# jaymarichua/Applestar

Hardware: AMD Instinct MI355X
Metric: learner samples/sec (AlphaStar policy) (higher is better)
Workload: dtype fp32

## Files before the change

applestar_amd/csrc/bindings.cpp:

```cpp
#include <cstring>
#include <cstdlib>
#include <map>
#include <string>
#include <torch/extension.h>
#include <c10/hip/HIPStream.h>
#include <c10/hip/HIPGuard.h>

#include "kernels.h"

namespace {

hipStream_t stream() { return c10::hip::getCurrentHIPStream().stream(); }

int dt(const at::Tensor& t) {
  if (t.scalar_type() == at::kFloat) return as::DT_F32;
  if (t.scalar_type() == at::kBFloat16) return as::DT_BF16;
  TORCH_CHECK(false, "applestar_amd: unsupported dtype ", t.scalar_type());
}

void check_cuda(const at::Tensor& t, const char* name) {
  TORCH_CHECK(t.is_cuda(), "applestar_amd: ", name, " must be a GPU tensor");
  TORCH_CHECK(t.is_contiguous(), "applestar_amd: ", name, " must be contiguous");
}

// ... 2298 lines not shown
    const at::Tensor& s = srcs[i];
    TORCH_CHECK(d.is_cuda() && s.is_cuda() && d.device() == s.device(), "multi_strided_copy: GPU tensors");
    TORCH_CHECK(d.is_contiguous(), "multi_strided_copy: contiguous destination");
    TORCH_CHECK((d.scalar_type() == at::kFloat || d.scalar_type() == at::kBFloat16) &&
                (s.scalar_type() == at::kFloat || s.scalar_type() == at::kBFloat16), "multi_strided_copy: fp32/bf16");
    const int64_t* sp = spec.data() + 9 * i;
    int64_t n = 1, lo = sp[8], hi = sp[8];
    for (int k = 0; k < 4; ++k) {
      TORCH_CHECK(sp[k] >= 1, "multi_strided_copy: sizes >= 1");
      n *= sp[k];
      const int64_t reach = (sp[k] - 1) * sp[4 + k];
      if (reach < 0) lo += reach; else hi += reach;
    }
    TORCH_CHECK(n == d.numel() && n < (int64_t{1} << 31), "multi_strided_copy: spec / destination size");
    int64_t extent = 1;
    for (int64_t k = 0; k < s.dim(); ++k) extent += (s.size(k) - 1) * s.stride(k);
    TORCH_CHECK(lo >= 0 && hi < extent, "multi_strided_copy: spec reaches outside the source");
    const int t = a.ntensors++;
    a.src[t] = s.data_ptr();
    a.dst[t] = d.data_ptr();
    a.n[t] = static_cast<int>(n);
    for (int k = 0; k < 4; ++k) {
      a.size[t][k] = static_cast<int>(sp[k]);
      a.stride[t][k] = sp[4 + k];
    }
    a.base[t] = sp[8];
    const bool tiled = sp[0] == 1 && sp[1] == 1 && sp[6] == 1 && sp[7] > 1 && n >= (1 << 16);
    a.dts[t] = static_cast<unsigned char>((s.scalar_type() == at::kFloat ? 1 : 0) | (d.scalar_type() == at::kFloat ? 2 : 0) |
                                          (tiled ? 4 : 0));
    const int64_t chunks = tiled ? ((sp[2] + 63) / 64) * ((sp[3] + 127) / 128) : (n + as::kCopyChunk - 1) / as::kCopyChunk;
    a.chunk_start[t + 1] = a.chunk_start[t] + static_cast<int>(chunks);
    if (a.ntensors == as::kSCopyMaxT) flush();
  }
  flush();
}

at::Tensor pointwise_conv(const at::Tensor& x, const at::Tensor& w, const c10::optional<at::Tensor>& bias, int64_t act) {
  check_cuda(x, "x");
  check_cuda(w, "w");
  TORCH_CHECK(x.scalar_type() == at::kBFloat16 && x.dim() == 2, "pointwise: x [P, cin] bf16");
  TORCH_CHECK(w.scalar_type() == at::kFloat && w.dim() == 2 && w.size(1) == x.size(1), "pointwise: w fp32 [cout, cin]");
  const int64_t P = x.size(0), cin = x.size(1), cout = w.size(0);
  TORCH_CHECK(as::pointwise_supported(static_cast<int>(cin), static_cast<int>(cout)), "pointwise: channels");
  const float* bp = nullptr;
  if (bias.has_value()) {
    check_cuda(*bias, "bias");
    TORCH_CHECK(bias->scalar_type() == at::kFloat && bias->numel() == cout, "pointwise: bias fp32 [cout]");
    bp = bias->data_ptr<float>();
  }
  c10::hip::HIPGuard g(x.device().index());
  auto y = at::empty({P, cout}, x.options());
  as::pointwise_conv(x.data_ptr(), w.data_ptr<float>(), bp, y.data_ptr(), P, static_cast<int>(cin),
                     static_cast<int>(cout), static_cast<int>(act), stream());
  return y;
}

void register_codec(pybind11::module& m);

PYBIND11_MODULE(TORCH_EXTENSION_NAME, m) {
  m.doc() = "applestar_amd HIP kernels for gfx950 (MI355X)";
  register_codec(m);
  m.def("layer_norm_fwd", &layer_norm_fwd);
  m.def("layer_norm_bwd", &layer_norm_bwd, py::arg("dy"), py::arg("xin"), py::arg("y"), py::arg("w"), py::arg("mean"),
        py::arg("rstd"), py::arg("dx_dtype"), py::arg("act"), py::arg("mask_src") = py::none());
  m.def("reverse_scan", &reverse_scan);
  m.def("col_sum", &col_sum);
  m.def("multi_logp", &multi_logp);
  m.def("presplit_b", &presplit_b, py::arg("b"), py::arg("trans") = false, py::arg("out") = py::none());
  m.def("gemm_f32_psb_supported", &gemm_f32_psb_supported);
  m.def("multi_presplit", &multi_presplit);
  m.def("conv3x3_f32_psb_supported", &conv3x3_f32_psb_supported);
  m.def("conv3x3_f32_psb", &conv3x3_f32_psb, py::arg("x"), py::arg("wsplit"), py::arg("Cout"),
        py::arg("bias") = py::none(), py::arg("res") = py::none(), py::arg("res2") = py::none(),
        py::arg("mask") = py::none(), py::arg("act") = 0);
  m.def("conv3x3_f32_v2", &conv3x3_f32_v2, py::arg("x"), py::arg("wsplit"), py::arg("Cout"),
        py::arg("bias") = py::none(), py::arg("res") = py::none(), py::arg("res2") = py::none(),
        py::arg("mask") = py::none(), py::arg("act") = 0, py::arg("variant") = 0);
  m.def("conv3x3_f32_halo_supported", &conv3x3_f32_halo_supported);
  m.def("conv3x3_f32_halo", &conv3x3_f32_halo, py::arg("x"), py::arg("wsplit"), py::arg("Cout"),
        py::arg("bias") = py::none(), py::arg("res") = py::none(), py::arg("res2") = py::none(),
        py::arg("mask") = py::none(), py::arg("act") = 0);
  m.def("conv_halo_f32_mode", &as::conv_halo_f32_mode);
  m.def("set_conv_halo_f32_mode", &as::set_conv_halo_f32_mode);
  m.def("gemm_f32_psb", &gemm_f32_psb, py::arg("a"), py::arg("bsplit"), py::arg("N"), py::arg("K"),
        py::arg("bias") = py::none(), py::arg("res") = py::none(), py::arg("act") = 0, py::arg("variant") = 0);
  m.def("entity_pack", &entity_pack);
  m.def("embed_relu_fwd", &embed_relu_fwd);
  m.def("embed_relu_bwd", &embed_relu_bwd, py::arg("dout"), py::arg("out"), py::arg("idx"), py::arg("V"),
        py::arg("ordered") = false);
  m.def("gated_residual_fwd", &gated_residual_fwd, py::arg("y"), py::arg("g"), py::arg("sp"), py::arg("x"),
        py::arg("post") = py::none());
  m.def("gated_residual_bwd", &gated_residual_bwd, py::arg("dout"), py::arg("y"), py::arg("g"), py::arg("sp"),
        py::arg("out"), py::arg("xin") = py::none());
  m.def("lnlstm_fwd", &lnlstm_fwd, py::arg("xp"), py::arg("h0"), py::arg("c0"), py::arg("wT"),
        py::arg("lnh_w"), py::arg("lnh_b"), py::arg("lnc_w"), py::arg("lnc_b"),
        py::arg("eps"), py::arg("want_bf16") = false);
  m.def("lnlstm_bwd", &lnlstm_bwd);
  m.def("entity_embed_fwd", &entity_embed_fwd);
  m.def("entity_onehot", &entity_onehot);
  m.def("upsample2x_fwd", &upsample2x_fwd);
  m.def("upsample2x_bwd", &upsample2x_bwd, py::arg("dy"), py::arg("mask") = py::none());
  m.def("entity_embed_wgrad", &entity_embed_wgrad);
  m.def("mm_k32", &mm_k32);
  m.def("spatial_embed_fwd", &spatial_embed_fwd, py::arg("planes"), py::arg("effects"), py::arg("w_dense"),
        py::arg("bias"), py::arg("rows"), py::arg("ex"), py::arg("ey"), py::arg("entity_num"), py::arg("out_dtype"),
        py::arg("ordered") = false);
  m.def("spatial_gather_rows", &spatial_gather_rows, py::arg("dpre"), py::arg("ex"), py::arg("ey"),
        py::arg("entity_num"), py::arg("N"), py::arg("gate") = py::none());
  m.def("spatial_dense_input", &spatial_dense_input);
  m.def("spatial_dense_wgrad", &spatial_dense_wgrad, py::arg("planes"), py::arg("effects"), py::arg("dpre"),
        py::arg("gate") = py::none());
  m.def("varlen_attn_fwd", &varlen_attn_fwd);
  m.def("varlen_attn_bwd", &varlen_attn_bwd);
  m.def("varlen_attn_fwd_f32", &varlen_attn_fwd_f32);
  m.def("conv3x3_f32_epi2", &conv3x3_f32_epi2);
  m.def("conv3x3_f32_epi2_supported", &conv3x3_f32_epi2_supported);
  m.def("conv3x3_f32", &conv3x3_f32);
  m.def("fused_clip_adam", &fused_clip_adam);
  m.def("head_sample", &head_sample);
  m.def("target_unit_sample", &target_unit_sample);
  m.def("fused_adam_chunk", &as::fused_adam_chunk);
  m.def("wgrad_f32", &wgrad_f32, py::arg("dy"), py::arg("x"), py::arg("cin"), py::arg("want_bias"),
        py::arg("out") = py::none());
  m.def("gemm_f32", &gemm_f32);
  m.def("gemm_bf16_small", &gemm_bf16_small);
  m.def("gemm_bf16", &gemm_bf16);
  m.def("small_gemm", &small_gemm);
  m.def("small_wgrad", &small_wgrad);
  m.def("small_gemm_splitk", &small_gemm_splitk);
  m.def("f32_mfma_mode", &as::f32_mfma_mode);
  m.def("set_f32_pipe_variant", &as::set_f32_pipe_variant);
  m.def("set_f32_conv_variant", &as::set_f32_conv_variant);
  m.def("set_f32_mfma_mode", &as::set_f32_mfma_mode);
  m.def("conv3x3_f32_supported", &as::conv3x3_f32_supported);
  m.def("varlen_attn_bwd_f32", &varlen_attn_bwd_f32);
  m.def("attn_f32_variant", [](int64_t v) { return static_cast<int64_t>(as::attn_f32_variant(static_cast<int>(v))); });
  m.def("su_sample", &su_sample);
  m.def("segment_copy", &segment_copy);
  m.def("conv_wt", &conv_wt);
  m.def("upconv1_fwd", &upconv1_fwd);
  m.def("upconv1_bwd", &upconv1_bwd, py::arg("x_nhwc"), py::arg("w"), py::arg("dy"), py::arg("relu_mask") = false);
  m.def("maxpool2_fwd", &maxpool2_fwd);
  m.def("maxpool2_bwd", &maxpool2_bwd, py::arg("dy"), py::arg("pos"), py::arg("H"), py::arg("W"),
        py::arg("mask") = py::none());
  m.def("maxpool2_bwd_relu", &maxpool2_bwd_relu);
  m.def("spatial_embed_pool_fwd", &spatial_embed_pool_fwd, py::arg("planes"), py::arg("effects"), py::arg("w_dense"),
        py::arg("bias"), py::arg("rows"), py::arg("ex"), py::arg("ey"), py::arg("entity_num"),
        py::arg("ordered") = false);
  m.def("spatial_pool_supported", [](int64_t h, int64_t w) { return as::spatial_pool_supported(static_cast<int>(h), static_cast<int>(w)); });
  m.def("segment_sum", &segment_sum);
  m.def("spatial_dense_wgrad_pooled", &spatial_dense_wgrad_pooled);
  m.def("spatial_gather_rows_pooled", &spatial_gather_rows_pooled);
  m.def("entity_mean_pool", &entity_mean_pool);
  m.def("table_grad", &table_grad, py::arg("src"), py::arg("idx"), py::arg("V"), py::arg("ordered") = false);
  m.def("gather_steps_fwd", &gather_steps_fwd);
  m.def("gather_steps_bwd", &gather_steps_bwd);
  m.def("scatter_conn_fwd", &scatter_conn_fwd);
  m.def("scatter_conn_bwd", &scatter_conn_bwd);
  m.def("conv3x3_fwd", &conv3x3_fwd);
  m.def("wgrad", &wgrad, py::arg("dy"), py::arg("x"), py::arg("cin"), py::arg("want_bias"),
        py::arg("bf16_out") = false);
  m.def("pointwise_conv", &pointwise_conv);
  m.def("pointwise_supported", [](int64_t ci, int64_t co) { return as::pointwise_supported(static_cast<int>(ci), static_cast<int>(co)); });
  m.def("lstm_split_error", &lstm_split_error);
  m.def("lstm_split_flag", &lstm_split_flag);
  m.def("multi_copy", &multi_copy);
// ... 29 lines not shown
```

applestar_amd/csrc/conv_tap.h:

```cpp
#pragma once
#include "common.h"

namespace as {

__device__ __forceinline__ int conv_tap_mask(long m, long M, int HW, int H, int W) {
  int ok = 0;
  if (m < M) {
    const int rem = static_cast<int>(m % HW);
    const int yy = rem / W, xx = rem - yy * W;
#pragma unroll
    for (int t = 0; t < 9; ++t) {
      const int y2 = yy + t / 3 - 1, x2 = xx + t % 3 - 1;
      ok |= (y2 >= 0 && y2 < H && x2 >= 0 && x2 < W) << t;
    }
  }
  return ok;
}

struct ConvTap {
  int tap, c0, shift;
  __device__ __forceinline__ bool in(int mask) const { return (mask >> tap) & 1; }
  __device__ __forceinline__ int offset(bool ok, int pix, int Cin, int c, int es) const {
    return ok ? ((pix + shift) * Cin + c0 + c) * es : kOOB;
  }
};

__device__ __forceinline__ ConvTap conv_tap(int k0, int Cin, int W) {
  const int tap = k0 / Cin;
  return ConvTap{tap, k0 - tap * Cin, (tap / 3 - 1) * W + (tap % 3 - 1)};
}

}
```

applestar_amd/csrc/kernels.h:

```cpp
#pragma once
#include <hip/hip_runtime.h>
#include <stdint.h>

namespace as {

enum DType : int { DT_F32 = 0, DT_BF16 = 1 };
enum SrcType : int { SRC_U8 = 0, SRC_I8 = 1, SRC_I16 = 2, SRC_I32 = 3, SRC_I64 = 4, SRC_F16 = 5, SRC_F32 = 6 };
enum FieldKind : int { FIELD_ONE_HOT = 0, FIELD_BINARY = 1, FIELD_SCALAR = 2 };

constexpr int kMaxFields = 40;
struct EntityFields {
  const void* ptr[kMaxFields];
  int dtype[kMaxFields];
  int kind[kMaxFields];
  int offset[kMaxFields];
  int width[kMaxFields];
  int n;
};

void layer_norm_fwd(const void* x, int x_dt, const void* res, int res_dt, const float* w, const float* b,
                    void* y, int y_dt, float* xsum, float* mean, float* rstd, long rows, int cols, float eps,
                    int act, hipStream_t s);
void layer_norm_bwd(const void* dy, int dy_dt, const void* xin, int xin_dt, const void* y, int y_dt,
                    const float* w, const float* mean, const float* rstd, void* dx, int dx_dt,
                    float* dw_part, float* db_part, long rows, int cols, int act, int nblk, hipStream_t s,
                    const float* msrc = nullptr, float* dxm = nullptr);
void column_reduce(const float* part, float* out, int nrows, int cols, hipStream_t s);
void entity_pack(const void* num, bool num64, int B, int N, long total, bool* valid, int64_t* flat, int64_t* seg,
                 int* cu, hipStream_t s);
void embed_relu_fwd(const void* table, int dt, const void* idx, int idt, void* out, long U, int V, int D,
                    hipStream_t s);
void embed_relu_bwd(const void* dout, const void* out, int dt, const void* idx, int idt, float* dtab, long U, int V,
                    int D, bool direct, hipStream_t s);
void column_reduce_bf16(const float* part, void* out, int nrows, int cols, hipStream_t s);
int layer_norm_bwd_blocks(long rows);

void reverse_scan(const float* a, const float* b, const float* init, float* y, int K, int T, int B,
                  hipStream_t s);

void gated_residual_fwd(const void* y, const void* g, const float* sp, const void* x, const void* post, void* out,
                        int dt, long n, hipStream_t s);
int vsp_in_channels();
int vsp_out_channels();
void vsp_fwd(const void* sc, const void* own, const void* enemy, const float* w, const float* b, void* out, long P,
             hipStream_t s, int dt = DT_BF16);
int vsp_bwd_blocks(long P);
void vsp_pool_fwd(const void* sc, const void* own, const void* enemy, const float* w, const float* b, void* pooled,
                  uint8_t* pos, int B, int H, int W, hipStream_t s, int dt = DT_BF16);
void vsp_pool_bwd(const void* dpooled, const uint8_t* pos, const void* pooled, const void* sc, const void* own,
                  const void* enemy, const float* w, void* dsc, float* part, int B, int H, int W, int nblk,
                  hipStream_t s, int dt = DT_BF16);
void vsp_bwd(const void* dout, const void* out, const void* sc, const void* own, const void* enemy, const float* w,
             void* dsc, float* part, long P, int nblk, hipStream_t s, int dt = DT_BF16);
bool loc_in_supported(int C, int P);
void loc_in_fwd(const void* y0, const void* p, const float* wp, void* out, long npix, int HW, hipStream_t s);
int loc_in_bwd_blocks(long npix);
void loc_in_bwd(const void* dy, const void* y, const void* p, const float* wp, void* dym, void* dp, float* part,
                long npix, int HW, int nblk, hipStream_t s);
void gated_residual_bwd(const void* dout, const void* y, const void* g, const float* sp, const void* out,
                        const void* xin, int dt, void* dy, void* dg, void* dx, float* dsp_part, long n, int nblk,
                        hipStream_t s);
int elementwise_blocks(long n);

bool lnlstm_supported(int H);
struct LstmSplit {
  unsigned long long* slab;
  int* err;
};
void lnlstm_fwd(const float* xp, const float* h0, const float* c0, const void* wT, int w_dt, const float* lnh_w,
                const float* lnh_b, const float* lnc_w, const float* lnc_b, int T, int B, int H, float eps, float* out,
                float* c_all, float* xhat_h, float* rstd_h, float* gates, float* xhat_c, float* rstd_c, float* hT,
                float* cT, hipStream_t s, const LstmSplit* split = nullptr, unsigned short* out_bf16 = nullptr);
void lnlstm_bwd(const float* dout, const float* dhT, const float* dcT, const float* gates, const float* c_all,
                const float* xhat_c, const float* rstd_c, const float* xhat_h, const float* rstd_h, const void* w,
                int w_dt, const float* lnh_w, const float* lnc_w, int T, int B, int H, float* dgates, float* dhg,
                float* dc_ln, float* dh0, float* dc0, hipStream_t s, const LstmSplit* split = nullptr);

void entity_embed_fwd(const EntityFields& f, const int64_t* index, const void* wT, int w_dt, const float* bias,
                      void* out, int out_dt, long T, hipStream_t s);
int entity_wgrad_chunks(long T);
void entity_embed_wgrad(const EntityFields& f, const int64_t* index, const void* dout, const void* out, int dt,
                        float* part, long T, int K_in, int nchunk, hipStream_t s);
void entity_onehot(const EntityFields& f, const int64_t* index, void* X, int x_dt, long T, int K_in, hipStream_t s);

struct SpatialPlanes {
  const uint8_t* height;
  const uint8_t* plane[6];
  const int16_t* effect[6];
};
void upsample2x_fwd(const void* x, void* y, int dt, int B, int H, int W, int C, hipStream_t s);
void upsample2x_bwd(const void* dy, void* dx, int dt, int B, int H, int W, int C, hipStream_t s,
                    const void* mask = nullptr);
void spatial_effect_bits(const SpatialPlanes& sp, uint8_t* bits, int B, int L, int HW, hipStream_t s);
void spatial_dense(const SpatialPlanes& sp, const uint8_t* bits, const float* wd, const float* bias, float* pre, long npix,
                   hipStream_t s);
void spatial_dense_input(const SpatialPlanes& sp, const uint8_t* bits, void* X, int x_dt, long npix, hipStream_t s);
void scatter_add_rows(const void* rows, int dt, const uint8_t* ex, const uint8_t* ey, const int64_t* entity_num,
                      float* pre, int B, int N, int H, int W, hipStream_t s);
void gather_rows(const void* dpre, const void* gate, int dt, const uint8_t* ex, const uint8_t* ey,
                 const int64_t* entity_num, void* drows, int B, int N, int H, int W, hipStream_t s);
void relu_cast(const float* x, void* y, int dt, long n, hipStream_t s);
void spatial_embed_fused(const SpatialPlanes& sp, const float* wd, const float* bias, const void* rows, int rows_dt,
                         const uint8_t* ex, const uint8_t* ey, const int64_t* entity_num, void* out, int out_dt, int B,
                         int N, int H, int W, int L, hipStream_t s, bool ordered = false);
bool spatial_pool_supported(int H, int W);
void spatial_embed_pool(const SpatialPlanes& sp, const float* wd, const float* bias, const void* rows, const uint8_t* ex,
                        const uint8_t* ey, const int64_t* entity_num, void* pooled, uint8_t* pos, int B, int N, int H,
                        int W, int L, hipStream_t s, bool f32 = false, bool ordered = false);
int spatial_wgrad_blocks(int B);
void spatial_dense_wgrad(const SpatialPlanes& sp, const void* dpre, const void* gate, int dt, float* part, int B, int H,
// ... 4 lines not shown
                        const int64_t* entity_num, float* drows, int B, int N, int H, int W, hipStream_t s);

void varlen_attn_fwd(const void* qkv, const int* cu, void* out, float* lse2, int S, int max_len, int H, long Ttot,
                     float scale, hipStream_t s);
void varlen_attn_bwd(const void* qkv, const void* out, const void* dout, const float* lse2, const int* cu, void* dqkv,
                     float* delta, int S, int max_len, int H, long Ttot, float scale, hipStream_t s);
void varlen_attn_fwd_f32(const float* qkv, const int* cu, float* out, float* lse2, int S, int max_len, int H, long Ttot,
                         float scale, hipStream_t s);
int attn_f32_variant(int v);
void varlen_attn_bwd_f32(const float* qkv, const float* out, const float* dout, const float* lse2, const int* cu,
                         float* dqkv, float* delta, int S, int max_len, int H, long Ttot, float scale, hipStream_t s);

}

namespace as {
void su_sample(const void* key, int key_dt, long key_bstride, const float* c0, const float* u, const int64_t* entity_num,
               const uint8_t* su_mask, const uint16_t* wf, const float* bf, const float* wq2, const float* bq2,
               const float* wih, const float* whh, const float* lni_w, const float* lni_b, const float* lnh_w,
               const float* lnh_b, const float* lnc_w, const float* lnc_b, const float* we1, const float* be1,
               float inv_temp, float eps, int B, int n1_stride, int max_steps, int extra_units, float* logits,
               int64_t* results, float* logp, int64_t* su_num, float* emb, float* extra, hipStream_t s);
}

namespace as {
void segment_copy(const uint8_t* arena, uint8_t* out, const int64_t* seg, long nseg, hipStream_t s);
void conv_wt(const uint16_t* w, uint16_t* out, int cout, int cin, long s0, long s1, long s2, long s3,
             hipStream_t s);
}

namespace as {
int upconv1_channels();
long upconv1_tiles(int B, int Hl, int Wl);
void upconv1_fwd(const void* x, int x_dt, const float* w, const float* bias, float* y, int B, int Hl, int Wl,
                 hipStream_t s);
void upconv1_bwd(const void* x, int x_dt, const float* w, const float* dy, void* dx, float* part, float* dwb, int B,
                 int Hl, int Wl, hipStream_t s, bool relu_mask = false);
}

namespace as {
void maxpool2_fwd(const void* x, void* y, uint8_t* pos, int dt, int B, int H, int W, int C, hipStream_t s);
void maxpool2_bwd(const void* dy, const uint8_t* pos, void* dx, int dt, int B, int H, int W, int C, hipStream_t s,
                  const void* mask = nullptr);
void maxpool2_bwd_relu(const void* dy, const uint8_t* pos, const void* y, void* dx, int B, int H, int W, int C,
                       hipStream_t s, bool f32 = false);
void segment_sum(const void* x, int dt, const int* cu, float* out, int S, int C, hipStream_t s);
void entity_mean_pool(const void* x, int dt, const bool* valid, const void* num, bool num64, void* out, int B, int N,
                      int C, hipStream_t s);
int ln_affine_slices(long R);
void ln_affine_grads(const float* dy, const float* xh, float* part, long R, int C, hipStream_t s);
void table_grad(const void* src, int dt, const int64_t* idx, float* out, long U, int V, int D, hipStream_t s);

bool conv3x3_supported(int Cin, int Cout);
void conv3x3_fwd(const void* x, const void* w, const float* bias, const void* res, void* out, int B, int H, int W,
                 int Cin, int Cout, int act, hipStream_t s);

bool conv3x3_f32_supported(int Cin, int Cout);
void conv3x3_f32_fwd(const float* x, const float* w, const float* bias, const float* res, float* out, int B, int H,
                     int W, int Cin, int Cout, int act, hipStream_t s);
bool conv3x3_f32_epi2_supported(int Cin, int Cout);
void conv3x3_f32_fwd_epi2(const float* x, const float* w, const float* res, const float* res2, long res2_rows,
                          const float* mask, float* out, int B, int H, int W, int Cin, int Cout, hipStream_t s);
int wgrad_f32_splits(long R, int N, int K);
void set_f32_pipe_variant(int v);
int f32_conv_variant();
void set_f32_conv_variant(int v);
int f32_mfma_mode();
void set_f32_mfma_mode(int mode);
void small_nt(const void* a, const void* b, const float* bias, const void* res, const void* amask, int mask_mode,
              void* out, long M, int N, int K, int act, bool bf16, hipStream_t s);
int small_nt_splits(long M, int N, int K);
void small_nt_splitk(const void* a, const void* b, const float* bias, float* part, int S, void* out, long M, int N,
                     int K, int act, bool bf16, hipStream_t s);
void small_tn(const void* dy, const void* x, const void* ymask, int mask_mode, void* dw, void* db, long R, int N,
              int K, bool bf16_in, bool bf16_out, hipStream_t s);
void gemm_bf16_small(const void* a, const void* b, const float* bias, const void* res, void* out, long M, int N, int K,
                     int act, hipStream_t s);
bool gemm_f32_is_small(long M, int N);
void gemm_bf16(const void* a, const void* b, const float* bias, const void* res, void* out, long M, int N, int K,
               int act, hipStream_t s);
void gemm_f32(const float* a, const float* b, const float* bias, const float* res, float* out, long M, int N, int K,
              int act, hipStream_t s);
void wgrad_f32(const float* dy, const float* x, float* dw_part, float* db_part, long part_stride, long R, int N, int K,
               int H, int W, int Cin, int S, hipStream_t st);

void head_sample(const void* logits, int logits_dt, long ld_logits, int B, int C, float inv_t, const uint8_t* mask,
                 long mask_ld, const int64_t* lens, const float* u, const void* table, int table_dt,
                 const float* tbias, int D, float* out_logits, int64_t* action, float* emb, hipStream_t s);
void target_unit_sample(const void* e, int e_dt, const float* w1, const float* b1, const float* w2, const float* b2,
                        const void* key, int key_dt, int B, int N, const int64_t* lens, float inv_t, const float* u,
                        float* out_logits, int64_t* action, hipStream_t s);

int fused_adam_chunk();
void fused_clip_adam(const void* table, const long* chunks, int nchunks, int ntensors, float* part,
                     const float* gate, float* norm_out, float max_norm, float* mom, float* scale, float* mom_init,
                     const float* hp, float lr_bc1, float b1, float b2, float inv_sqrt_bc2, float eps, float wd,
                     int decoupled, hipStream_t s);

int wgrad_splits(long R, int N, int K);

constexpr int kCopyMaxT = 64;
constexpr long kCopyChunk = 8192;
constexpr long kCopyRawChunk = 16384;
struct CopyArgs {
  int ntensors;
  int chunk_start[kCopyMaxT + 1];
  const void* src[kCopyMaxT];
  void* dst[kCopyMaxT];
  long n[kCopyMaxT];
  unsigned char dts[kCopyMaxT];
};
void multi_copy(const CopyArgs& a, hipStream_t s);

constexpr int kColMaxP = 32;
struct ColSumArgs {
  int npieces;
  long rows;
  int block_start[kColMaxP + 1];
  float* dst[kColMaxP];
  int dld[kColMaxP], doff[kColMaxP], width[kColMaxP], nsrc[kColMaxP];
  const float* src[kColMaxP][3];
  int sld[kColMaxP][3], soff[kColMaxP][3];
};
void col_sum(const ColSumArgs& a, hipStream_t s);

constexpr int kLogpMaxH = 8;
struct LogpArgs {
  int nheads;
  long row_start[kLogpMaxH + 1];
  const void* logits[kLogpMaxH];
  const int64_t* action[kLogpMaxH];
  float* out[kLogpMaxH];
  int cols[kLogpMaxH];
  unsigned char bf16[kLogpMaxH];
  long blk_start[kLogpMaxH + 1];
  unsigned char big[kLogpMaxH];
};
void multi_logp(const LogpArgs& a, hipStream_t s);

long presplit_b_bytes(int N, int K);
void presplit_b(const float* b, int N, int K, bool trans, void* out, hipStream_t s);
bool gemm_f32_psb_supported(long M, int N, int K);
constexpr int kPresplitMax = 48;
struct PresplitArgs {
  int n;
  int block_start[kPresplitMax + 1];
  const float* src[kPresplitMax];
  void* dst[kPresplitMax];
  int N[kPresplitMax], K[kPresplitMax];
  unsigned char trans[kPresplitMax];
};
void multi_presplit(const PresplitArgs& a, hipStream_t s);
void gemm_f32_psb(const float* a, const void* bsplit, const float* bias, const float* res, float* out, long M, int N,
                  int K, int act, int variant, hipStream_t s);
bool conv3x3_f32_psb_supported(long M, int Cin, int Cout);
void conv3x3_f32_psb(const float* x, const void* wsplit, const float* bias, const float* res, const float* res2,
                     long res2_rows, const float* mask, float* out, int B, int H, int W, int Cin, int Cout, int act,
                     hipStream_t s);
void conv3x3_f32_psb_stream(const float* x, const void* wsplit, const float* bias, const float* res,
                            const float* res2, long res2_rows, const float* mask, float* out, int B, int H, int W,
                            int Cin, int Cout, int act, hipStream_t s);
void conv3x3_f32_v2(const float* x, const void* wsplit, const float* bias, const float* res, const float* res2,
                    long res2_rows, const float* mask, float* out, int B, int H, int W, int Cin, int Cout, int act,
                    int variant, hipStream_t s);
void gemm_f32_v2(const float* a, const void* bsplit, const float* bias, const float* res, float* out, long M, int N,
                 int K, int act, int variant, hipStream_t s);
bool conv3x3_f32_halo_supported(int H, int W, int Cin, int Cout);
// ... 140 lines not shown
```

applestar_amd/csrc/kernels/pool_reduce.hip:

```cpp
#include <algorithm>

#include "../common.h"
#include "../kernels.h"

namespace as {
namespace {

struct V8 {
  float v[8];
};

template <typename T> __device__ __forceinline__ V8 load8(const T* p);
template <> __device__ __forceinline__ V8 load8<bf16_t>(const bf16_t* p) {
  const uint4 u = *reinterpret_cast<const uint4*>(p);
  const uint32_t w[4] = {u.x, u.y, u.z, u.w};
  V8 r;
#pragma unroll
  for (int j = 0; j < 4; ++j) {
    r.v[2 * j] = __uint_as_float(w[j] << 16);
    r.v[2 * j + 1] = __uint_as_float(w[j] & 0xffff0000u);
  }
  return r;
}
template <> __device__ __forceinline__ V8 load8<float>(const float* p) {
// ... 455 lines not shown
    if (num64) AS_EMP(float, int64_t); else AS_EMP(float, int);
  }
#undef AS_EMP
}

void segment_sum(const void* x, int dt, const int* cu, float* out, int S, int C, hipStream_t s) {
  if (S == 0) return;
  if (dt == DT_BF16)
    hipLaunchKernelGGL(segment_sum_kernel<bf16_t>, dim3(S), dim3(256), 0, s, static_cast<const bf16_t*>(x), cu, out, C);
  else
    hipLaunchKernelGGL(segment_sum_kernel<float>, dim3(S), dim3(256), 0, s, static_cast<const float*>(x), cu, out, C);
}

void table_grad(const void* src, int dt, const int64_t* idx, float* out, long U, int V, int D, hipStream_t s) {
  const long n = U * D;
  if (n == 0) return;
  long blocks = (n + 4095) / 4096;
  if (blocks > 256) blocks = 256;
  if (blocks < 1) blocks = 1;
  const size_t lds = static_cast<size_t>(V) * D * sizeof(float);
  if (dt == DT_BF16)
    hipLaunchKernelGGL(table_grad_kernel<bf16_t>, dim3(static_cast<unsigned>(blocks)), dim3(256), lds, s,
                       static_cast<const bf16_t*>(src), idx, out, U, V, D);
  else
    hipLaunchKernelGGL(table_grad_kernel<float>, dim3(static_cast<unsigned>(blocks)), dim3(256), lds, s,
                       static_cast<const float*>(src), idx, out, U, V, D);
}

#define AS_EMB_IDX(IDT, BODY)                                      \
  switch (IDT) {                                                   \
    case 0: { using I = int64_t; BODY; } break;                    \
    case 1: { using I = int32_t; BODY; } break;                    \
    case 2: { using I = int16_t; BODY; } break;                    \
    case 3: { using I = uint8_t; BODY; } break;                    \
    default: { using I = int8_t; BODY; } break;                    \
  }

void embed_relu_fwd(const void* table, int dt, const void* idx, int idt, void* out, long U, int V, int D,
                    hipStream_t s) {
  const long n = U * D;
  if (n == 0) return;
  const unsigned blocks = static_cast<unsigned>(std::min<long>((n + 255) / 256, 1024));
  if (dt == DT_BF16) {
    AS_EMB_IDX(idt, hipLaunchKernelGGL((embed_relu_fwd_kernel<bf16_t, I>), dim3(blocks), dim3(256), 0, s,
                                       static_cast<const bf16_t*>(table), static_cast<const I*>(idx),
                                       static_cast<bf16_t*>(out), U, V, D))
  } else {
    AS_EMB_IDX(idt, hipLaunchKernelGGL((embed_relu_fwd_kernel<float, I>), dim3(blocks), dim3(256), 0, s,
                                       static_cast<const float*>(table), static_cast<const I*>(idx),
                                       static_cast<float*>(out), U, V, D))
  }
}

void embed_relu_bwd(const void* dout, const void* out, int dt, const void* idx, int idt, float* dtab, long U, int V,
                    int D, bool direct, hipStream_t s) {
  const long n = U * D;
  long blocks = direct ? 1 : std::min<long>(std::max<long>((n + 1023) / 1024, 1), 256);
  const size_t lds = static_cast<size_t>(V) * D * sizeof(float);
  if (dt == DT_BF16) {
    AS_EMB_IDX(idt, hipLaunchKernelGGL((embed_relu_bwd_kernel<bf16_t, I>), dim3(static_cast<unsigned>(blocks)),
                                       dim3(256), lds, s, static_cast<const bf16_t*>(dout),
                                       static_cast<const bf16_t*>(out), static_cast<const I*>(idx), dtab, U, V, D,
                                       direct ? 1 : 0))
  } else {
    AS_EMB_IDX(idt, hipLaunchKernelGGL((embed_relu_bwd_kernel<float, I>), dim3(static_cast<unsigned>(blocks)),
                                       dim3(256), lds, s, static_cast<const float*>(dout),
                                       static_cast<const float*>(out), static_cast<const I*>(idx), dtab, U, V, D,
                                       direct ? 1 : 0))
  }
}
#undef AS_EMB_IDX

void entity_pack(const void* num, bool num64, int B, int N, long total, bool* valid, int64_t* flat, int64_t* seg,
                 int* cu, hipStream_t s) {
  if (B == 0) return;
  if (num64)
    hipLaunchKernelGGL(entity_pack_kernel<int64_t>, dim3(B), dim3(256), 0, s, static_cast<const int64_t*>(num), B, N,
                       total, valid, flat, seg, cu);
  else
    hipLaunchKernelGGL(entity_pack_kernel<int>, dim3(B), dim3(256), 0, s, static_cast<const int*>(num), B, N, total,
                       valid, flat, seg, cu);
}

void column_reduce(const float* part, float* out, int nrows, int cols, hipStream_t s) {
  if (nrows <= 1024) {
    hipLaunchKernelGGL(column_reduce_kernel<float>, dim3((cols + 63) / 64), dim3(1024), 0, s, part, out, nrows, cols,
                       static_cast<long>(cols));
    return;
  }
  const int nchunk = (nrows + 255) / 256;
  hipLaunchKernelGGL(column_reduce_chunk_kernel, dim3((cols + 63) / 64, nchunk), dim3(256), 0, s,
                     const_cast<float*>(part), nrows, cols);
  hipLaunchKernelGGL(column_reduce_kernel<float>, dim3((cols + 63) / 64), dim3(1024), 0, s, part, out, nchunk, cols,
                     256L * cols);
}

void column_reduce_bf16(const float* part, void* out, int nrows, int cols, hipStream_t s) {
  hipLaunchKernelGGL(column_reduce_kernel<bf16_t>, dim3((cols + 63) / 64), dim3(1024), 0, s, part,
                     static_cast<bf16_t*>(out), nrows, cols, static_cast<long>(cols));
}

int ln_affine_slices(long R) { return static_cast<int>((R + kAffRows - 1) / kAffRows); }

void ln_affine_grads(const float* dy, const float* xh, float* part, long R, int C, hipStream_t s) {
  const int S = ln_affine_slices(R);
  if (S == 0 || C == 0) return;
  hipLaunchKernelGGL(ln_affine_grads_kernel, dim3((C + 63) / 64, S), dim3(256), 0, s, dy, xh, part, R, C);
}

}
```

applestar_amd/csrc/kernels/wgrad_f32.hip:

```cpp
#include "../common.h"
#include "../kernels.h"
#include "../split_mfma.h"
#include "../f32_pipe.h"

namespace as {
namespace {

typedef __attribute__((ext_vector_type(16))) float f16v;

template <int BN_, int BK_>
struct WgF32Cfg {
  static constexpr int BN = BN_, BK = BK_, BR = 32, NT = 256;
  static constexpr int WN = BN_ >= 64 ? 2 : 1, WK = 4 / WN;
  static constexpr int TN = BN / WN, TK = BK / WK;
  static constexpr int FN = TN / 32, FK = TK / 32;
  static constexpr int PA = BN + 4, PB = BK + 4;
  static constexpr int CHA = BN / 4, CHB = BK / 4;
  static constexpr int A_IT = BR * CHA / NT, B_IT = BR * CHB / NT;
  static constexpr int STAGE = BR * (PA + PB);
  static_assert(A_IT * NT == BR * CHA && B_IT * NT == BR * CHB, "tile / thread mismatch");
};

template <int BN, int BK, bool CONV, int SPLIT>
__global__ __launch_bounds__(256) void wgrad_f32_kernel(const float* __restrict__ dy, const float* __restrict__ x,
// ... 585 lines not shown
  if constexpr (BK == 128) {
    if (f32_mfma_mode() == 1 && wgrad_stg() && (BN == 128 || wgrad_stg_narrow())) {
      hipLaunchKernelGGL((wgrad_f32_stg_kernel<BN, CONV>), dim3(static_cast<unsigned>(nwg)), dim3(256), 0, st, dy, x,
                         dwp, dbp, ps, R, N, K, H, W, Cin, rps, tn, tk);
      return;
    }
  }
  if constexpr (BN >= 32 && (BK <= 128 || (BN == 128 && BK == 256))) {
    if (f32_mfma_mode() == 1 && !(BN == 32 && wgrad_f32_pipe32_off())) {
      hipLaunchKernelGGL((wgrad_f32_pipe_kernel<BN, BK, CONV, 3>), dim3(static_cast<unsigned>(nwg)), dim3(256), 0, st,
                         dy, x, dwp, dbp, ps, R, N, K, H, W, Cin, rps, tn, tk);
      return;
    }
  }
  if (f32_mfma_mode())
    hipLaunchKernelGGL((wgrad_f32_kernel<BN, BK, CONV, 1>), dim3(static_cast<unsigned>(nwg)), dim3(256), 0, st, dy, x,
                       dwp, dbp, ps, R, N, K, H, W, Cin, rps, tn, tk);
  else
    hipLaunchKernelGGL((wgrad_f32_kernel<BN, BK, CONV, 0>), dim3(static_cast<unsigned>(nwg)), dim3(256), 0, st, dy,
                       x, dwp, dbp, ps, R, N, K, H, W, Cin, rps, tn, tk);
}

int pick(int n) { return n <= 32 ? 32 : (n <= 64 ? 64 : 128); }
bool wgrad32_bk256() {
  static const bool on = [] {
    const char* e = std::getenv("APPLESTAR_WGRAD32_BK");
    return e != nullptr && e[0] == '2';
  }();
  return on;
}
bool wgrad_wide() {
  static const bool on = [] {
    const char* e = std::getenv("APPLESTAR_WGRAD_WIDE");
    return e != nullptr && e[0] == '1';
  }();
  return on;
}
int pick_k(int k, int bn) {
  if (bn == 32) return (k >= 256 && wgrad32_bk256()) ? 256 : 128;
  if (bn == 128 && k >= 256 && wgrad_wide() && f32_mfma_mode() == 1) return 256;
  return k <= 64 ? 64 : 128;
}

}

long wgrad_f32_target_wg() {
  static const long v = [] {
    const char* e = std::getenv("APPLESTAR_WGRAD_F32_WG");
    const long x = e ? std::atol(e) : 3072;
    return x >= 64 ? x : 3072;
  }();
  return v;
}

long wgrad_f32_small_r_rows() {
  static const long v = [] {
    const char* e = std::getenv("APPLESTAR_WGRAD_SMALL_R");
    return e ? std::atol(e) : 48L;
  }();
  return v;
}

int wgrad_f32_splits(long R, int N, int K) {
  const int bn = pick(N), bk = pick_k(K, bn);
  const long tiles = static_cast<long>((N + bn - 1) / bn) * ((K + bk - 1) / bk);
  const long target = wgrad_f32_target_wg();
  long S = (target + tiles - 1) / tiles;
  const long small = wgrad_f32_small_r_rows();
  const long max_s = R < 2048 ? (small > 0 && R >= 2 * small ? R / small : 1)
                              : (R + 127) / 128;
  if (S > max_s) S = max_s;
  const long max_part = (16L << 20) / (static_cast<long>(N) * K);
  if (S > max_part) S = max_part;
  if (S < 1) S = 1;
  if (S > 4096) S = 4096;
  return static_cast<int>(S);
}

void wgrad_f32(const float* dy, const float* x, float* dw_part, float* db_part, long part_stride, long R, int N, int K,
               int H, int W, int Cin, int S, hipStream_t st) {
  long rps = (R + S - 1) / S;
  rps = (rps + 31) / 32 * 32;
  const bool conv = Cin > 0;
  const int bn = pick(N), bk = pick_k(K, bn);
#define AS_WGF(BNv, BKv)                                                                   \
  if (bn == BNv && bk == BKv) {                                                            \
    if (conv) launch<BNv, BKv, true>(dy, x, dw_part, db_part, part_stride, R, N, K, H, W, Cin, S, rps, st); \
    else launch<BNv, BKv, false>(dy, x, dw_part, db_part, part_stride, R, N, K, H, W, Cin, S, rps, st);     \
    return;                                                                                \
  }
  AS_WGF(128, 128) AS_WGF(128, 64) AS_WGF(64, 128) AS_WGF(64, 64) AS_WGF(32, 128) AS_WGF(32, 256) AS_WGF(128, 256)
#undef AS_WGF
}

}
```

Measured before the change: 8393.

## Add halo-ring LDS conv3x3 weight-gradient kernel for fp32 split-MFMA

Adds a specialised conv3x3 weight-gradient kernel that stages input rows into an LDS ring buffer with a halo. All nine taps then reuse the same staged input via shifted offsets instead of reloading an im2col-style K slice per tap. It uses transposed LDS reads and split-bf16 MFMA with double-buffered dy tiles. It is selected by default (mode 4) only for N not equal to 32 or 64, with N%128==0, W<=80 and the 3-way split MFMA mode active. The trade-off is extra LDS pressure, nine accumulators per thread and more code paths to keep correct.

```diff
diff --git a/applestar_amd/csrc/bindings.cpp b/applestar_amd/csrc/bindings.cpp
--- a/applestar_amd/csrc/bindings.cpp
+++ b/applestar_amd/csrc/bindings.cpp
@@ -2404,6 +2404,10 @@
         py::arg("mask") = py::none(), py::arg("act") = 0);
   m.def("conv_halo_f32_mode", &as::conv_halo_f32_mode);
   m.def("set_conv_halo_f32_mode", &as::set_conv_halo_f32_mode);
+  m.def("conv_wgrad_halo_f32_mode", &as::conv_wgrad_halo_f32_mode);
+  m.def("set_conv_wgrad_halo_f32_mode", &as::set_conv_wgrad_halo_f32_mode);
+  m.def("conv_wgrad_f32_halo_selected", &as::conv_wgrad_f32_halo_selected, py::arg("cout"), py::arg("h"), py::arg("w"),
+        py::arg("cin"));
   m.def("gemm_f32_psb", &gemm_f32_psb, py::arg("a"), py::arg("bsplit"), py::arg("N"), py::arg("K"),
         py::arg("bias") = py::none(), py::arg("res") = py::none(), py::arg("act") = 0, py::arg("variant") = 0);
   m.def("entity_pack", &entity_pack);
diff --git a/applestar_amd/csrc/conv_tap.h b/applestar_amd/csrc/conv_tap.h
--- a/applestar_amd/csrc/conv_tap.h
+++ b/applestar_amd/csrc/conv_tap.h
@@ -3,18 +3,21 @@
 
 namespace as {
 
-__device__ __forceinline__ int conv_tap_mask(long m, long M, int HW, int H, int W) {
+__device__ __forceinline__ int conv_tap_mask_yx(int yy, int xx, int H, int W) {
   int ok = 0;
-  if (m < M) {
-    const int rem = static_cast<int>(m % HW);
-    const int yy = rem / W, xx = rem - yy * W;
 #pragma unroll
-    for (int t = 0; t < 9; ++t) {
-      const int y2 = yy + t / 3 - 1, x2 = xx + t % 3 - 1;
-      ok |= (y2 >= 0 && y2 < H && x2 >= 0 && x2 < W) << t;
-    }
+  for (int t = 0; t < 9; ++t) {
+    const int y2 = yy + t / 3 - 1, x2 = xx + t % 3 - 1;
+    ok |= (y2 >= 0 && y2 < H && x2 >= 0 && x2 < W) << t;
   }
   return ok;
+}
+
+__device__ __forceinline__ int conv_tap_mask(long m, long M, int HW, int H, int W) {
+  if (m >= M) return 0;
+  const int rem = static_cast<int>(m % HW);
+  const int yy = rem / W;
+  return conv_tap_mask_yx(yy, rem - yy * W, H, W);
 }
 
 struct ConvTap {
diff --git a/applestar_amd/csrc/kernels.h b/applestar_amd/csrc/kernels.h
--- a/applestar_amd/csrc/kernels.h
+++ b/applestar_amd/csrc/kernels.h
@@ -25,7 +25,7 @@
                     const float* w, const float* mean, const float* rstd, void* dx, int dx_dt,
                     float* dw_part, float* db_part, long rows, int cols, int act, int nblk, hipStream_t s,
                     const float* msrc = nullptr, float* dxm = nullptr);
-void column_reduce(const float* part, float* out, int nrows, int cols, hipStream_t s);
+void column_reduce(float* part, float* out, int nrows, int cols, hipStream_t s);
 void entity_pack(const void* num, bool num64, int B, int N, long total, bool* valid, int64_t* flat, int64_t* seg,
                  int* cu, hipStream_t s);
 void embed_relu_fwd(const void* table, int dt, const void* idx, int idt, void* out, long U, int V, int D,
@@ -196,6 +196,12 @@
               int act, hipStream_t s);
 void wgrad_f32(const float* dy, const float* x, float* dw_part, float* db_part, long part_stride, long R, int N, int K,
                int H, int W, int Cin, int S, hipStream_t st);
+int conv_wgrad_halo_f32_mode();
+void set_conv_wgrad_halo_f32_mode(int mode);
+bool conv_wgrad_f32_halo_supported(int N, int H, int W, int Cin);
+bool conv_wgrad_f32_halo_selected(int N, int H, int W, int Cin);
+void conv_wgrad_f32_halo(const float* dy, const float* x, float* dw_part, float* db_part, long part_stride, long R,
+                         int N, int K, int H, int W, int Cin, int S, long rows_per_split, hipStream_t st);
 
 void head_sample(const void* logits, int logits_dt, long ld_logits, int B, int C, float inv_t, const uint8_t* mask,
                  long mask_ld, const int64_t* lens, const float* u, const void* table, int table_dt,
diff --git a/applestar_amd/csrc/kernels/conv_wgrad_f32_halo.hip b/applestar_amd/csrc/kernels/conv_wgrad_f32_halo.hip
--- /dev/null
+++ b/applestar_amd/csrc/kernels/conv_wgrad_f32_halo.hip
@@ -0,0 +1,269 @@
+#include <cstdlib>
+
+#include "../common.h"
+#include "../kernels.h"
+#include "../split_mfma.h"
+#include "../f32_pipe.h"
+#include "../conv_tap.h"
+
+namespace as {
+namespace {
+
+using pipe::f16v;
+
+constexpr int kWgBN = 128, kWgCC = 32, kWgRS = 16, kWgMaxW = 80;
+
+typedef short s16x4 __attribute__((ext_vector_type(4)));
+typedef __attribute__((address_space(3))) s16x4 lds_s16x4;
+
+template <int WMAX>
+struct WgHaloCfg {
+  static constexpr int SA = kWgBN * 2 + 64, SX = kWgCC * 2;
+  static constexpr int NRING = 2 * kWgRS + 2 * WMAX + 2 <= 128 ? 128 : 256;
+  static constexpr int PA = kWgRS * SA;
+  static constexpr int PX = (NRING + 1) * SX;
+  static constexpr int SMEM = 6 * PA + 3 * PX;
+  static_assert(2 * kWgRS + 2 * WMAX + 2 <= NRING && 2 * SMEM <= 160 * 1024, "ring size / two workgroups per CU");
+};
+
+__device__ __forceinline__ s16x4 tr_read(const char* p) {
+  return __builtin_amdgcn_ds_read_tr16_b64_v4i16((lds_s16x4*)p);
+}
+
+__device__ __forceinline__ u32v4 tr_frag(const char* p0, const char* p1) {
+  const uint2 lo = __builtin_bit_cast(uint2, tr_read(p0)), hi = __builtin_bit_cast(uint2, tr_read(p1));
+  return u32v4{lo.x, lo.y, hi.x, hi.y};
+}
+
+__device__ __forceinline__ void split_store(char* plane0, int plane_bytes, int off, const uint4 v) {
+  uint2 s0, s1, s2;
+  split4(v, s0, s1, s2);
+  *reinterpret_cast<uint2*>(plane0 + off) = s0;
+  *reinterpret_cast<uint2*>(plane0 + plane_bytes + off) = s1;
+  *reinterpret_cast<uint2*>(plane0 + 2 * plane_bytes + off) = s2;
+}
+
+template <int WMAX>
+__global__ __launch_bounds__(256, 2) void conv_wgrad_f32_halo_kernel(const float* __restrict__ dy,
+                                                                     const float* __restrict__ x,
+                                                                     float* __restrict__ dw_part,
+                                                                     float* __restrict__ db_part, long part_stride,
+                                                                     long R, int N, int K, int H, int W, int Cin,
+                                                                     long rows_per_split, int tiles_n, int chunks) {
+  using C = WgHaloCfg<WMAX>;
+  constexpr int RS = kWgRS, BN = kWgBN, CC = kWgCC, SA = C::SA, SX = C::SX;
+  constexpr int RINGB = C::NRING * SX;
+  __shared__ __attribute__((aligned(16))) char smem[C::SMEM];
+  char* const pa = smem;
+  char* const px = smem + 6 * C::PA;
+
+  const int wg = pipe::xcd_remap();
+  const int ch = wg % chunks;
+  const int tn = (wg / chunks) % tiles_n;
+  const int s = wg / (chunks * tiles_n);
+  const int n0 = tn * BN, c0 = ch * CC;
+  const long r_begin = static_cast<long>(s) * rows_per_split;
+  const long r_end = r_begin + rows_per_split < R ? r_begin + rows_per_split : R;
+  const int tid = threadIdx.x, lane = tid & 63, wid = __builtin_amdgcn_readfirstlane(tid >> 6);
+  const int l32 = lane & 31, h = lane >> 5;
+  const int HW = H * W;
+  const __amdgpu_buffer_rsrc_t yr =
+      __builtin_amdgcn_make_buffer_rsrc(const_cast<float*>(dy), 0, static_cast<int>(R * N * 4), 0x00020000);
+  const __amdgpu_buffer_rsrc_t xr =
+      __builtin_amdgcn_make_buffer_rsrc(const_cast<float*>(x), 0, static_cast<int>(R * Cin * 4), 0x00020000);
+  const int nrows = r_end > r_begin ? static_cast<int>(r_end - r_begin) : 0;
+  const int nsteps = (nrows + RS - 1) / RS;
+
+  const int a_q = tid & 31, a_row = tid >> 5;
+  const bool a_colok = n0 + 4 * a_q < N;
+  int a_base[2], a_lim[2];
+#pragma unroll
+  for (int i = 0; i < 2; ++i) {
+    a_base[i] = static_cast<int>(((r_begin + a_row + 8 * i) * N + n0 + 4 * a_q) * 4);
+    a_lim[i] = a_colok ? nrows - (a_row + 8 * i) : 0;
+  }
+  const int a_step = RS * N * 4;
+  const int x_q = tid & 7, x_row = (tid >> 3) & 15;
+  const bool x_colok = c0 + 4 * x_q < Cin, x_wave = wid < 2;
+  const int x_base = static_cast<int>(((r_begin + W + 1 + x_row) * Cin + c0 + 4 * x_q) * 4);
+  const long x_left = R - (r_begin + W + 1 + x_row);
+  const int x_lim = (x_colok && x_wave && x_left > 0) ? static_cast<int>(x_left) : 0;
+  const int x_step = RS * Cin * 4;
+  const bool do_bias = db_part != nullptr && ch == 0;
+  const int b_col = n0 + (tid & 127), b_h = tid >> 7;
+  const int b_base = static_cast<int>(((r_begin + 8 * b_h) * N + b_col) * 4);
+  const int b_lim = b_col < N ? nrows - 8 * b_h : 0;
+  float rb[8], bsum = 0.f;
+  uint4 ra[2], rx;
+  auto load_stage = [&](int j) {
+    if (do_bias) {
+#pragma unroll
+      for (int q = 0; q < 8; ++q)
+        rb[q] = __uint_as_float(__builtin_amdgcn_raw_buffer_load_b32(
+            yr, j * RS + q < b_lim ? b_base + j * a_step + q * N * 4 : kOOB, 0, 0));
+    }
+#pragma unroll
+    for (int i = 0; i < 2; ++i) {
+      const auto v =
+          __builtin_amdgcn_raw_buffer_load_b128(yr, j * RS < a_lim[i] ? a_base[i] + j * a_step : kOOB, 0, 0);
+      ra[i] = make_uint4(v[0], v[1], v[2], v[3]);
+    }
+    const auto v = __builtin_amdgcn_raw_buffer_load_b128(xr, j * RS < x_lim ? x_base + j * x_step : kOOB, 0, 0);
+    rx = make_uint4(v[0], v[1], v[2], v[3]);
+  };
+  auto add_bias = [&]() {
+    if (do_bias) {
+#pragma unroll
+      for (int q = 0; q < 8; ++q) bsum += rb[q];
+    }
+  };
+  const int a_dst = a_row * SA + a_q * 8;
+  const int x_dst0 = (2 * (W + 1) + x_row) * SX + x_q * 8;
+  auto store_stage = [&](int j) {
+#pragma unroll
+    for (int i = 0; i < 2; ++i) split_store(pa + (j & 1) * 3 * C::PA, C::PA, a_dst + 8 * i * SA, ra[i]);
+    add_bias();
+    if (x_wave) split_store(px, C::PX, (x_dst0 + j * RS * SX) & (RINGB - 1), rx);
+  };
+
+  const int g = lane >> 4, tq = (lane >> 2) & 3, tp = lane & 3;
+  const int rr0 = 8 * (g >> 1) + tq;
+  const int a_off = rr0 * SA + (32 * wid + 16 * (g & 1) + 4 * tp) * 2;
+  const int x_col = (16 * (g & 1) + 4 * tp) * 2;
+  const int x_off0 = (W + 1 + rr0) * SX + x_col;
+  const int x_zero = RINGB + x_col;
+  int shb[9];
+#pragma unroll
+  for (int t = 0; t < 9; ++t) shb[t] = ((t / 3 - 1) * W + (t % 3 - 1)) * SX;
+  int py[2], pxx[2];
+#pragma unroll
+  for (int r = 0; r < 2; ++r) {
+    const int rem = static_cast<int>((r_begin + rr0 + 4 * r) % HW);
+    py[r] = rem / W;
+    pxx[r] = rem - py[r] * W;
+  }
+  const int adv = RS % HW, adv_y = adv / W, adv_x = adv - adv_y * W;
+
+  f16v acc[9];
+#pragma unroll
+  for (int t = 0; t < 9; ++t)
+#pragma unroll
+    for (int e = 0; e < 16; ++e) acc[t][e] = 0.f;
+
+  for (int i = tid; i < 3 * SX / 4; i += 256)
+    *reinterpret_cast<unsigned*>(px + (i / (SX / 4)) * C::PX + RINGB + (i % (SX / 4)) * 4) = 0u;
+  load_stage(0);
+  {
+    const int npieces = (RS + 2 * W + 2) * (CC / 4);
+    for (int piece = tid; piece < npieces; piece += 256) {
+      const int row = piece >> 3;
+      const long pix = r_begin - (W + 1) + row;
+      const bool ok = x_colok && pix >= 0 && pix < R;
+      const auto v = __builtin_amdgcn_raw_buffer_load_b128(
+          xr, ok ? (static_cast<int>(pix) * Cin + c0 + 4 * x_q) * 4 : kOOB, 0, 0);
+      split_store(px, C::PX, row * SX + x_q * 8, make_uint4(v[0], v[1], v[2], v[3]));
+    }
+  }
+  {
+#pragma unroll
+    for (int i = 0; i < 2; ++i) split_store(pa, C::PA, a_dst + 8 * i * SA, ra[i]);
+    add_bias();
+  }
+  __syncthreads();
+
+  for (int j = 0; j < nsteps; ++j) {
+    const bool more = j + 1 < nsteps;
+    if (more) load_stage(j + 1);
+    int ok[2];
+#pragma unroll
+    for (int r = 0; r < 2; ++r) {
+      ok[r] = conv_tap_mask_yx(py[r], pxx[r], H, W);
+      pxx[r] += adv_x;
+      py[r] += adv_y;
+      if (pxx[r] >= W) { pxx[r] -= W; ++py[r]; }
+      if (py[r] >= H) py[r] -= H;
+    }
+    const char* ap = pa + (j & 1) * 3 * C::PA + a_off;
+    Split3 fa;
+#pragma unroll
+    for (int p = 0; p < 3; ++p) fa.p[p] = tr_frag(ap + p * C::PA, ap + p * C::PA + 4 * SA);
+    const int xs = x_off0 + j * RS * SX;
+    auto read_x = [&](int t) {
+      const int m0 = __builtin_amdgcn_sbfe(ok[0], t, 1), m1 = __builtin_amdgcn_sbfe(ok[1], t, 1);
+      const int o0 = (((xs + shb[t]) & (RINGB - 1)) & m0) | (x_zero & ~m0);
+      const int o1 = (((xs + 4 * SX + shb[t]) & (RINGB - 1)) & m1) | (x_zero & ~m1);
+      Split3 f;
+#pragma unroll
+      for (int p = 0; p < 3; ++p) f.p[p] = tr_frag(px + p * C::PX + o0, px + p * C::PX + o1);
+      return f;
+    };
+    Split3 fb[2];
+    fb[0] = read_x(0);
+#pragma unroll
+    for (int t = 0; t < 9; ++t) {
+      if (t + 1 < 9) fb[(t + 1) & 1] = read_x(t + 1);
+      __builtin_amdgcn_sched_barrier(0);
+      acc[t] = mfma_x6(fa, fb[t & 1], acc[t]);
+      __builtin_amdgcn_sched_barrier(0);
+    }
+    if (more) store_stage(j + 1);
+    __syncthreads();
+  }
+
+  float* outp = dw_part + static_cast<long>(s) * part_stride;
+  const int c = c0 + l32;
+  if (c < Cin) {
+#pragma unroll
+    for (int t = 0; t < 9; ++t)
+#pragma unroll
+      for (int e = 0; e < 16; ++e) {
+        const int n = n0 + 32 * wid + (e & 3) + 8 * (e >> 2) + 4 * h;
+        if (n < N) outp[static_cast<long>(n) * K + t * Cin + c] = acc[t][e];
+      }
+  }
+  if (do_bias) {
+    float* red = reinterpret_cast<float*>(smem);
+    red[tid] = bsum;
+    __syncthreads();
+    if (b_h == 0 && b_col < N) db_part[static_cast<long>(s) * part_stride + b_col] = bsum + red[tid + 128];
+  }
+}
+
+template <int WMAX>
+void launch_wg_halo(const float* dy, const float* x, float* dwp, float* dbp, long ps, long R, int N, int K, int H,
+                    int W, int Cin, int S, long rps, hipStream_t st) {
+  const int tiles_n = (N + kWgBN - 1) / kWgBN, chunks = (Cin + kWgCC - 1) / kWgCC;
+  const long nwg = static_cast<long>(S) * tiles_n * chunks;
+  hipLaunchKernelGGL((conv_wgrad_f32_halo_kernel<WMAX>), dim3(static_cast<unsigned>(nwg)), dim3(256), 0, st, dy, x,
+                     dwp, dbp, ps, R, N, K, H, W, Cin, rps, tiles_n, chunks);
+}
+
+int& wg_halo_ref() {
+  static int v = [] {
+    const char* e = std::getenv("APPLESTAR_CONV_WGRAD_HALO_F32");
+    return e ? std::atoi(e) & 7 : 4;
+  }();
+  return v;
+}
+
+}
+
+int conv_wgrad_halo_f32_mode() { return wg_halo_ref(); }
+void set_conv_wgrad_halo_f32_mode(int mode) { wg_halo_ref() = mode & 7; }
+
+bool conv_wgrad_f32_halo_supported(int N, int H, int W, int Cin) {
+  return f32_mfma_mode() == 1 && H > 0 && W > 0 && W <= kWgMaxW && Cin > 0 && Cin % 16 == 0 && N > 0 && N % 128 == 0;
+}
+
+bool conv_wgrad_f32_halo_selected(int N, int H, int W, int Cin) {
+  const int bit = N == 32 ? 1 : (N == 64 ? 2 : 4);
+  return (conv_wgrad_halo_f32_mode() & bit) != 0 && conv_wgrad_f32_halo_supported(N, H, W, Cin);
+}
+
+void conv_wgrad_f32_halo(const float* dy, const float* x, float* dw_part, float* db_part, long part_stride, long R,
+                         int N, int K, int H, int W, int Cin, int S, long rows_per_split, hipStream_t st) {
+  if (W <= 40) launch_wg_halo<40>(dy, x, dw_part, db_part, part_stride, R, N, K, H, W, Cin, S, rows_per_split, st);
+  else launch_wg_halo<kWgMaxW>(dy, x, dw_part, db_part, part_stride, R, N, K, H, W, Cin, S, rows_per_split, st);
+}
+
+}
diff --git a/applestar_amd/csrc/kernels/pool_reduce.hip b/applestar_amd/csrc/kernels/pool_reduce.hip
--- a/applestar_amd/csrc/kernels/pool_reduce.hip
+++ b/applestar_amd/csrc/kernels/pool_reduce.hip
@@ -561,15 +561,15 @@
                        valid, flat, seg, cu);
 }
 
-void column_reduce(const float* part, float* out, int nrows, int cols, hipStream_t s) {
+void column_reduce(float* part, float* out, int nrows, int cols, hipStream_t s) {
   if (nrows <= 1024) {
     hipLaunchKernelGGL(column_reduce_kernel<float>, dim3((cols + 63) / 64), dim3(1024), 0, s, part, out, nrows, cols,
                        static_cast<long>(cols));
     return;
   }
   const int nchunk = (nrows + 255) / 256;
-  hipLaunchKernelGGL(column_reduce_chunk_kernel, dim3((cols + 63) / 64, nchunk), dim3(256), 0, s,
-                     const_cast<float*>(part), nrows, cols);
+  hipLaunchKernelGGL(column_reduce_chunk_kernel, dim3((cols + 63) / 64, nchunk), dim3(256), 0, s, part, nrows,
+                     cols);
   hipLaunchKernelGGL(column_reduce_kernel<float>, dim3((cols + 63) / 64), dim3(1024), 0, s, part, out, nchunk, cols,
                      256L * cols);
 }
diff --git a/applestar_amd/csrc/kernels/wgrad_f32.hip b/applestar_amd/csrc/kernels/wgrad_f32.hip
--- a/applestar_amd/csrc/kernels/wgrad_f32.hip
+++ b/applestar_amd/csrc/kernels/wgrad_f32.hip
@@ -691,6 +691,10 @@
   long rps = (R + S - 1) / S;
   rps = (rps + 31) / 32 * 32;
   const bool conv = Cin > 0;
+  if (conv && conv_wgrad_f32_halo_selected(N, H, W, Cin)) {
+    conv_wgrad_f32_halo(dy, x, dw_part, db_part, part_stride, R, N, K, H, W, Cin, S, rps, st);
+    return;
+  }
   const int bn = pick(N), bk = pick_k(K, bn);
 #define AS_WGF(BNv, BKv)                                                                   \
   if (bn == BNv && bk == BKv) {                                                            \
```

Result: faster. 8519 (median of 6 runs) (+1.5%).
